# izhengfan/se2lam

Measured on AMD Instinct MI355X. Metric: BA GN-iters/s (200 KF, 20k pts), higher is better.
Workload: dtype f64; 1 GPU; globalBA-window 200 KF / 20000 landmarks / 119817 EdgeSE2XYZ + 199 PreEdgeSE2, LM optimize(10) (config 4 formulation, SURVEY D3); parallelism=single GPU

## Files before the change

experiments/chol32_emu.cpp:

```cpp
#include "waveemu.h"

#include <cmath>
#include <cstdio>
#include <cstdlib>
#include <cstring>
#include <string>
#include <vector>

using std::min;
using std::max;
#define __host__
#define WAVE_LOCKSTEP() waveemu::wave_barrier()
#define SE2_WAIT_VM6(a, b, c, d, e, f) WAIT_VM()
static inline void WAIT_VM();
struct BaCtl { int done; };
static inline double bcast_lane(double v, int lane) { return waveemu_readlane(v, lane); }
static inline d2_t load_agent(const double* p) { return d2_t{p[0], p[1]}; }
struct PendingStore { double* p; d2_t v; };
static thread_local std::vector<PendingStore> g_pending[256];
static inline void store_agent(double* p, d2_t v) { g_pending[waveemu::g()->cur].push_back(PendingStore{p, v}); }
static inline void WAIT_VM() {
    std::vector<PendingStore>& q = g_pending[waveemu::g()->cur];
    for (const PendingStore& s : q) { s.p[0] = s.v.x; s.p[1] = s.v.y; }
    q.clear();
// ... 30 lines not shown
    std::printf("n = %d%s: ld %d, %d tile rows, %d block columns (%d on the longest chain), %d tasks of 256 threads\n", S.n, nd ? " (two arcs + separator)" : "", S.ld,
                S.nt, S.nbc, S.chain, ntask);
    std::vector<double> PUB(2 * (size_t)S.nt * S.nbc * kSlabs * kSlabDoubles + S.ld, 0.0), x(S.n, 0.0);
    std::vector<unsigned> flagA((size_t)S.nt * S.nbc * kSlabs, 0u), flagR((size_t)S.nt * S.nbc * kSlabs, 0u);
    double fail = 0.0;
    int rc = 0, same = 0;
    std::vector<double> x_first;
    for (unsigned seed = seed0; seed < seed0 + nseeds; ++seed) {
        std::fill(PUB.begin(), PUB.end(), 0.0);
        std::fill(x.begin(), x.end(), 0.0);
        double* YU = PUB.data() + 2 * (size_t)S.nt * S.nbc * kSlabs * kSlabDoubles;
        unsigned epoch = seed;
        unsigned long long sw = 0;
        static unsigned long long head = 0;
        auto task = [&]() {
            d_chol_tiles<false>(blockIdx.x, S.A.data(), PUB.data(), YU, S.ld, S.n, S.nbc, S.plan.tasks.data(), S.plan.deps.data(), nullptr, flagA.data(), flagR.data(),
                                &epoch, &fail, nullptr, nullptr, x.data(), nullptr, &head, ntask);
            WAIT_VM();
        };
        if (resident > 0)
            waveemu::run_grid(256, ntask, resident, seed, task);
        else
            for (int t = 0; t < ntask; ++t) sw += waveemu::run_group(256, t, ntask, seed * 7919u + t, task);
        const double res = chol_residual(S, x);
        std::printf("interleaving %u: %llu switches, |A x - b|_inf / |b|_inf = %.3e %s, failure flag %g\n", seed, sw, res, res < 1e-11 ? "(ok)" : "(MISMATCH)", fail);
        if (indefinite) {
            std::printf("  (indefinite system: the failure flag is %s)\n", fail == 1.0 ? "raised, as it must be" : "NOT raised");
            return fail == 1.0 ? 0 : 1;
        }
        if (!(res < 1e-11) || fail != 0.0) rc = 1;
        if (x_first.empty()) x_first = x;
// ... 7 lines not shown
```

experiments/waveemu/chol_host.h:

```cpp
#pragma once
#include <algorithm>
#include <cstdio>
#include <vector>

struct Plan {
    std::vector<int4> tasks;
    std::vector<int> deps;
};

inline Plan plan_from_pattern(std::vector<std::vector<char>> P, int nt, int nbc, int* chain_len) {
    for (int m = 0; m < nbc; ++m)
        for (int j = m + 1; j < nbc; ++j)
            if (P[j][m])
                for (int i = j; i < nt; ++i)
                    if (P[i][m]) P[i][j] = 1;
    std::vector<std::vector<char>> R(nbc, std::vector<char>(nbc, 0));
    for (int r = 0; r < nbc; ++r) {
        R[r][r] = 1;
        for (int j = r + 1; j < nbc; ++j)
            for (int m = r; m < j; ++m)
                if (R[r][m] && P[j][m]) { R[r][j] = 1; break; }
    }
    Plan p;
    auto add = [&](int kind, int i, int j, const std::vector<int>& d) {
        int4 t;
        t.x = i | (kind << 16); t.y = j; t.z = (int)p.deps.size();
        p.deps.insert(p.deps.end(), d.begin(), d.end());
        t.w = (int)p.deps.size();
        p.tasks.push_back(t);
    };
    std::vector<int> depth(nbc, 1);
    for (int j = 0; j < nbc; ++j) {
        for (int m = 0; m < j; ++m)
            if (P[j][m]) depth[j] = std::max(depth[j], depth[m] + 1);
        for (int i = j; i < nt; ++i) {
            if (i > j && !P[i][j]) continue;
            std::vector<int> d;
            for (int m = 0; m < j; ++m)
                if (P[j][m]) d.push_back(m | (i != j && P[i][m] ? 1 << 15 : 0));
            add(0, i, j, d);
        }
        for (int r = 0; r < j; ++r) {
            if (!R[r][j]) continue;
            std::vector<int> d;
            for (int m = 0; m < j; ++m)
                if (P[j][m]) d.push_back(m | (m >= r && R[r][m] ? 1 << 15 : 0));
            add(1, r, j, d);
        }
    }
    for (int r = 0; r < nbc; ++r) {
        std::vector<int> d;
        for (int j = r; j < nbc; ++j)
            if (R[r][j]) d.push_back(j);
        add(2, r, 0, d);
    }
    *chain_len = *std::max_element(depth.begin(), depth.end());
    return p;
}

struct CholSystem {
    int n, ld, nt, nbc, chain;
    std::vector<double> A, b;
    Plan plan;
};
inline CholSystem chol_system(int NB, int n_dense, int arc, int sep) {
    CholSystem S;
    const bool nd = arc > 0;
    const int n = S.n = nd ? NB * (2 * arc + sep) : n_dense;
    const int ld = S.ld = ((n + 1 + NB - 1) / NB) * NB, nt = S.nt = ld / NB, nbc = S.nbc = (n + NB - 1) / NB;
    std::vector<std::vector<char>> P(nt, std::vector<char>(nbc, 1));
    if (nd)
// ... 26 lines not shown
                if (S.A[(size_t)r * ld + c] != 0.0) { std::printf("the arcs are coupled?\n"); std::abort(); }
    S.plan = plan_from_pattern(P, nt, nbc, &S.chain);
    return S;
}
inline bool chol_system_from_file(int NB, const char* path, CholSystem& S) {
    FILE* f = std::fopen(path, "rb");
    int hdr[4];
    if (!f || std::fread(hdr, 4, 4, f) != 4) return false;
    S.n = hdr[0]; S.ld = hdr[1]; S.nt = S.ld / NB; S.nbc = (S.n + NB - 1) / NB; S.chain = 0;
    S.plan.tasks.resize(hdr[2]); S.plan.deps.resize(hdr[3]); S.A.resize((size_t)S.ld * S.ld); S.b.resize(S.n);
    bool ok = std::fread(S.plan.tasks.data(), sizeof(int4), hdr[2], f) == (size_t)hdr[2];
    ok = ok && std::fread(S.plan.deps.data(), 4, hdr[3], f) == (size_t)hdr[3];
    ok = ok && std::fread(S.A.data(), 8, S.A.size(), f) == S.A.size();
    std::fclose(f);
    for (int c = 0; ok && c < S.n; ++c) S.b[c] = S.A[(size_t)S.n * S.ld + c];
    return ok;
}
inline double chol_residual(const CholSystem& S, const std::vector<double>& x) {
    double worst = 0.0, scale = 0.0;
    for (int r = 0; r < S.n; ++r) {
        double a = -S.b[r];
        for (int c = 0; c < S.n; ++c) a += S.A[(size_t)r * S.ld + c] * x[c];
        if (!(std::fabs(a) <= worst)) worst = std::fabs(a);
        scale = std::fmax(scale, std::fabs(S.b[r]));
    }
    return worst / scale;
}
```

include/se2gpu.h:

```cpp
#ifndef SE2GPU_H
#define SE2GPU_H

#include <stddef.h>
#include <stdint.h>

#ifdef __cplusplus
extern "C" {
#endif

#define SE2GPU_OK 0
#define SE2GPU_ERR_INVALID (-1)
#define SE2GPU_ERR_NO_DEVICE (-2)
#define SE2GPU_ERR_HIP (-3)
#define SE2GPU_ERR_CAPACITY (-4)
#define SE2GPU_ERR_STATE (-5)

const char* se2gpu_last_error(void);
int se2gpu_device_count(void);
const char* se2gpu_version(void);

typedef struct se2gpu_orb se2gpu_orb;

typedef struct se2gpu_orb_params {
    int32_t nfeatures;
// ... 173 lines not shown
int se2gpu_ba_get_se2(se2gpu_ba* h, int id, double xyt[3]);
int se2gpu_ba_get_xyz(se2gpu_ba* h, int id, double xyz[3]);
int se2gpu_ba_get_all(se2gpu_ba* h, double* poses , double* lms );
double se2gpu_ba_chi2(se2gpu_ba* h);

int se2gpu_ba_debug_reduced_system(se2gpu_ba* h, double lambda, double* S, double* bs);
int se2gpu_ba_debug_solve(se2gpu_ba* h, double lambda, double* x, int* factor_ok);
int se2gpu_ba_debug_solver_path(const se2gpu_ba* h);
int se2gpu_ba_debug_linearize_counts(const se2gpu_ba* h, int* runs, int* skips, long long* twin_bytes);
int se2gpu_ba_debug_pool_sizes(int out2[2]);
int se2gpu_ba_debug_chol_verify(se2gpu_ba* h, unsigned long long* counts2, unsigned long long* records, int cap);
int se2gpu_ba_debug_solve_plan(int P, int D, const uint8_t* pattern, int allow_nd, int* nsys, int* nbc, int* depth, int* ntask,
                               int* ndep, int32_t* pose_off, int32_t* tasks4, int task_cap, int32_t* deps, int dep_cap);
int se2gpu_ba_debug_solve_plan_tile(int P, int D, const uint8_t* pattern, int allow_nd, int tile, int* nsys, int* nbc, int* depth, int* ntask,
                                    int* ndep, int32_t* pose_off, int32_t* tasks4, int task_cap, int32_t* deps, int dep_cap);

int se2gpu_triangulate(int n, const se2gpu_keypoint* kps_ref, const se2gpu_keypoint* kps_cur, int n_cur,
                       int32_t* match_idx, const uint8_t* has_observation, const float* P_ref, const float* P_cur,
                       const float* Ocam, float lower_depth, float upper_depth, int min_degree, float* pos_out,
                       uint8_t* good_parallax, int* n_good, int* n_tracked_old);

typedef struct se2gpu_track se2gpu_track;
int se2gpu_track_create(se2gpu_track** out);
void se2gpu_track_destroy(se2gpu_track* h);
int se2gpu_track_fundamental_mask(se2gpu_track* h, const float* pt1, const float* pt2, int n, uint8_t* mask,
                                  int* n_inliers);
int se2gpu_track_remove_outliers(se2gpu_track* h, const se2gpu_keypoint* kps1, int n1, const se2gpu_keypoint* kps2,
                                 int n2, int32_t* matches, int* n_inliers);
int se2gpu_track_last_ransac(const se2gpu_track* h, int info[4]);
int se2gpu_track_triangulate(se2gpu_track* h, int n, const se2gpu_keypoint* kps_ref, const se2gpu_keypoint* kps_cur,
// ... 103 lines not shown
```

se2lam_amd/capi.py:

```python
from __future__ import annotations

import ctypes as C
import os

import numpy as np

HERE = os.path.dirname(os.path.abspath(__file__))
LIB_PATH = os.path.join(HERE, "lib", "libse2gpu.so")

OK = 0
ERR_INVALID, ERR_NO_DEVICE, ERR_HIP, ERR_CAPACITY, ERR_STATE = -1, -2, -3, -4, -5


class Se2GpuError(RuntimeError):
    def __init__(self, code, msg):
        super().__init__(f"se2gpu error {code}: {msg}")
        self.code = code


class Keypoint(C.Structure):
    _fields_ = [("x", C.c_float), ("y", C.c_float), ("size", C.c_float), ("angle", C.c_float),
                ("response", C.c_float), ("octave", C.c_int32), ("class_id", C.c_int32)]


# ... 125 lines not shown
    "se2gpu_ba_optimize": (_I, [_VP, _I, _I, _PU8, _I, C.POINTER(BaStats)]),
    "se2gpu_ba_optimize_batch": (_I, [C.POINTER(_VP), _I, _I, _I, _PU8, C.POINTER(BaStats)]),
    "se2gpu_ba_last_batch_path": (_I, []),
    "se2gpu_ba_get_se2": (_I, [_VP, _I, _PD]),
    "se2gpu_ba_get_xyz": (_I, [_VP, _I, _PD]),
    "se2gpu_ba_get_all": (_I, [_VP, _PD, _PD]),
    "se2gpu_ba_chi2": (_D, [_VP]),
    "se2gpu_ba_debug_reduced_system": (_I, [_VP, _D, _PD, _PD]),
    "se2gpu_ba_debug_solve": (_I, [_VP, _D, _PD, C.POINTER(C.c_int)]),
    "se2gpu_ba_debug_solver_path": (_I, [_VP]),
    "se2gpu_ba_debug_linearize_counts": (_I, [_VP, C.POINTER(C.c_int), C.POINTER(C.c_int), C.POINTER(C.c_longlong)]),
    "se2gpu_ba_debug_chol_verify": (_I, [_VP, _VP, _VP, _I]),
    "se2gpu_ba_debug_pool_sizes": (_I, [_VP]),
    "se2gpu_ba_debug_solve_plan": (_I, [_I, _I, _VP, _I, _VP, _VP, _VP, _VP, _VP, _VP, _VP, _I, _VP, _I]),
    "se2gpu_ba_debug_solve_plan_tile": (_I, [_I, _I, _VP, _I, _I, _VP, _VP, _VP, _VP, _VP, _VP, _VP, _I, _VP, _I]),
    "se2gpu_triangulate": (_I, [_I, _VP, _VP, _I, _VP, _VP, _VP, _VP, _VP, C.c_float, C.c_float, _I, _VP, _VP,
                           C.POINTER(C.c_int), C.POINTER(C.c_int)]),
    "se2gpu_track_create": (_I, [C.POINTER(_VP)]),
    "se2gpu_track_destroy": (None, [_VP]),
    "se2gpu_track_fundamental_mask": (_I, [_VP, _VP, _VP, _I, _VP, C.POINTER(C.c_int)]),
    "se2gpu_track_remove_outliers": (_I, [_VP, _VP, _I, _VP, _I, _VP, C.POINTER(C.c_int)]),
    "se2gpu_track_last_ransac": (_I, [_VP, _VP]),
    "se2gpu_plane_motion_prior": (_I, [_VP, _VP, _D, _D, _D, _VP, _VP]),
    "se2gpu_track_pose_ba": (_I, [_VP, _VP, _VP, _VP, _I, _VP, _VP, _VP, _D, _D, _D, _D, _I, _VP, C.POINTER(BaStats)]),
    "se2gpu_track_triangulate": (_I, [_VP, _I, _VP, _VP, _I, _VP, _VP, _VP, _VP, _VP, C.c_float, C.c_float, _I, _VP, _VP,
                                 C.POINTER(C.c_int), C.POINTER(C.c_int)]),
    "se2gpu_ba_reduce_buffer_doubles": (_SZ, [_VP, _I]),
    "se2gpu_ba_exchange_doubles": (_SZ, [_I]),
    "se2gpu_ba_exchange_doubles_h": (_SZ, [_VP]),
    "se2gpu_ba_exchange_row": (_I, [_I, C.POINTER(C.c_size_t), C.POINTER(C.c_int)]),
# ... 187 lines not shown
```

se2lam_amd/csrc/ba.hip:

```cpp
#include <algorithm>
#include <atomic>
#include <chrono>
#include <cmath>
#include <cstdlib>
#include <functional>
#include <limits>
#include <mutex>
#include <thread>
#include <tuple>
#include <memory>
#include <unordered_map>

#include "common.h"
#include "se3_math.h"
#include "ba_device.h"
#include "ba3_device.h"
#include "ba_window.h"

using namespace se2gpu;
using namespace se2gpu::badev;

namespace {


// ... 940 lines not shown

constexpr int kVfyRecords = 64, kVfyChk = 8 + 8 * kVfyRecords;
__device__ inline unsigned long long wave_xor64(unsigned long long v) {
#pragma unroll
    for (int m = 1; m < 64; m <<= 1) v ^= (unsigned long long)__shfl_xor((long long)v, m);
    return v;
}
__device__ inline unsigned long long bits4(d2_t a, d2_t b) {
    return (unsigned long long)__double_as_longlong(a.x) ^ (unsigned long long)__double_as_longlong(a.y) ^
           (unsigned long long)__double_as_longlong(b.x) ^ (unsigned long long)__double_as_longlong(b.y);
}
template <bool VERIFY>
__device__ __forceinline__ void d_chol_tiles(const unsigned bx_dispatch, const double* __restrict__ A, double* __restrict__ PUB,
                                                     double* __restrict__ YU, int ld, int n,
                                                     int nbc, const int4* __restrict__ tasks, const int* __restrict__ deps,
                                                     const int* __restrict__ col_src,
                                                     unsigned* __restrict__ flagA, unsigned* __restrict__ flagR,
                                                     const unsigned* __restrict__ epoch_ptr, double* __restrict__ fail,
                                                     long long* __restrict__ dbg, const BaCtl* __restrict__ ctl,
                                                     double* __restrict__ xout, unsigned long long* __restrict__ vfy,
                                                     unsigned long long* __restrict__ head, int ntask) {
    if (ctl && ctl->done) return;
    __shared__ unsigned task_s;
    if (head) {
        if (threadIdx.x == 0) {
            const unsigned c = __hip_atomic_fetch_add(reinterpret_cast<unsigned*>(head), 1u, __ATOMIC_RELAXED, __HIP_MEMORY_SCOPE_AGENT);
            if (c == (unsigned)ntask - 1u) __hip_atomic_store(reinterpret_cast<unsigned*>(head), 0u, __ATOMIC_RELAXED, __HIP_MEMORY_SCOPE_AGENT);
            task_s = c;
        }
        __syncthreads();
// ... 6 lines not shown
    double (*Tb)[kNB + 2] = reinterpret_cast<double (*)[kNB + 2]>(LD);
    double (*Tc)[kNB + 2] = reinterpret_cast<double (*)[kNB + 2]>(LD + kTile);
    double (*Ta)[kNB + 2] = reinterpret_cast<double (*)[kNB + 2]>(LD + 2 * kTile);
    double (*COLV)[kNB] = reinterpret_cast<double (*)[kNB]>(LD + 3 * kTile);
    double* const DUMMY = LD + 3 * kTile + kNB * kNB;
    double (*MRC)[64] = reinterpret_cast<double (*)[64]>(LD + kTile);
    static_assert(16 * 64 <= kTile && 32 * 64 <= 2 * kTile, "rows 0..15 of MRC lie inside Tc, all of it inside Tc | Ta");
    __shared__ int ok_s, ready_s, loaded_s, slab_s[kSlabs];
    __shared__ int deps_s[64];
    const int tid = threadIdx.x;
    if (tid == 0) { ready_s = 0; loaded_s = 0; ok_s = 1; }
    if (tid < kSlabs) slab_s[tid] = 0;
    long long* stamp = dbg ? dbg + (size_t)bx * 16 : nullptr;
    if (stamp && tid == 0) stamp[0] = wall_clock64();
    const int4 tk = tasks[bx];
    if (tid < tk.w - tk.z && tid < 64) deps_s[tid] = deps[tk.z + tid];
    __syncthreads();
    if ((tk.x >> 16) == 2) {
        const int r = tk.x & 0xffff;
        const int it = n / kNB;
        const int row = tid / 8, c4 = (tid % 8) * 4;
        double acc = 0.0;
        for (int dq = tk.z; dq < tk.w; ++dq) {
            const int j = deps_s[dq - tk.z];
            if (tid == 0) {
                const bool lazy = dq + 1 < tk.w;
                bool ok = true;
                for (int sl = 0; sl < kSlabs; ++sl) {
                    ok = ok && spin_until(flagR + ((size_t)r * nbc + j) * kSlabs + sl, epoch, lazy);
                    ok = ok && spin_until((it == j ? flagR : flagA) + ((size_t)it * nbc + j) * kSlabs + sl, epoch, lazy);
// ... 37 lines not shown
#pragma unroll
    for (int v = 0; v < 4; ++v) {
        D0[v] = A[(size_t)(kNB * j + orow + 4 * v) * ld + kNB * j + ocol];
        if (!isR && !isDiag) T0[v] = A[(size_t)(kNB * i + orow + 4 * v) * ld + kNB * j + ocol];
    }
    const int sr = ln >> 1, sc = 8 * wv + 4 * (ln & 1);
    for (int dq = tk.z; dq < tk.w; ++dq) {
        const int dep = deps_s[dq - tk.z];
        const int m = dep & 0x7fff;
        const bool hasT = (dep >> 15) != 0;
        __syncthreads();
        if (!ok_s) {
            if (tid == 0) fail[0] = 1e6;
            return;
        }
        const bool lazy = dq + 1 < tk.w;
        const unsigned* f0 = flagA + ((size_t)j * nbc + m) * kSlabs + wv;
        const unsigned* f1 = hasT ? (isR ? flagR : flagA) + ((size_t)i * nbc + m) * kSlabs + wv : f0;
        const int need = dq - tk.z + 1;
        bool staged = false;
        int mult = 0;
        long long t0 = 0;
        while (mult < kSlabs) {
            unsigned v0 = 0, v1 = 0;
            if (!staged) { v0 = poll_agent(f0); v1 = poll_agent(f1); }
            bool progress = false;
            if (__hip_atomic_load(&slab_s[mult], __ATOMIC_ACQUIRE, __HIP_MEMORY_SCOPE_WORKGROUP) >= need) {
                const int k0 = 8 * mult + acol;
                const double b0 = Tb[qj + arow][k0], b1 = Tb[qj + arow][k0 + 4];
                const double c0 = Tc[qi + arow][k0], c1 = Tc[qi + arow][k0 + 4];
                const double a0 = Ta[qi + arow][k0], a1 = Ta[qi + arow][k0 + 4];
// ... 184 lines not shown
    if (!isR && i == n / kNB && lane == (isDiag ? 0 : kNB) + n % kNB) {
#pragma unroll
        for (int q = 0; q < 8; q += 2) store_agent(YU + c0 + cb + q, d2_t{m[q], m[q + 1]});
    }
    if (bad && isDiag && lane == 0) fail[0] = 1.0;
    asm volatile("s_waitcnt vmcnt(0)" ::: "memory");
    if (lane == 0)
        __hip_atomic_store((isR || isDiag ? flagR : flagA) + ((size_t)i * nbc + j) * kSlabs + w, epoch, __ATOMIC_RELAXED, __HIP_MEMORY_SCOPE_AGENT);
    if (stamp && lane == 0) stamp[12 + w] = wall_clock64();
    if (stamp && tid == 192) stamp[5] = wall_clock64();
}
template <bool VERIFY>
__global__ __launch_bounds__(256) void k_chol_tiles(const double* __restrict__ A, double* __restrict__ PUB,
                                                     double* __restrict__ YU, int ld, int n,
                                                     int nbc, const int4* __restrict__ tasks, const int* __restrict__ deps,
                                                     const int* __restrict__ col_src,
                                                     unsigned* __restrict__ flagA, unsigned* __restrict__ flagR,
                                                     const unsigned* __restrict__ epoch_ptr, double* __restrict__ fail,
                                                     long long* __restrict__ dbg, const BaCtl* __restrict__ ctl,
                                                     double* __restrict__ xout, unsigned long long* __restrict__ vfy,
                                                     unsigned long long* __restrict__ head, int ntask) {
    d_chol_tiles<VERIFY>(blockIdx.x, A, PUB, YU, ld, n, nbc, tasks, deps, col_src, flagA, flagR, epoch_ptr, fail, dbg, ctl, xout, vfy, head, ntask);
}

__global__ __launch_bounds__(256) void k_chol_apply(const double* __restrict__ A, const double* __restrict__ R, int ld,
                                                     int n, double* __restrict__ x, const BaCtl* __restrict__ ctl,
                                                     const int* __restrict__ col_src) {
    if (ctl && ctl->done) return;
    const int r = blockIdx.x * 4 + threadIdx.x / 64;
    const int lane = threadIdx.x & 63;
    if (r >= n) return;
    const double* y = A + (size_t)n * ld;
    double acc = 0.0;
    for (int c = r + lane; c < n; c += 64) acc += R[(size_t)r * ld + c] * y[c];
    acc = wave_sum(acc);
    const int dst = col_src ? col_src[r] : r;
    if (lane == 0 && dst >= 0) x[dst] = acc;
// ... 1359 lines not shown
    DevBuf<int4> grp;
    int nwg_off = 0, grp_cap_wg = 0;
    DevBuf<uint8_t> garena;
    DevBuf<int> plan_np, plan_base, plan_key0, plan_key1, plan_idx, plan_hist, plan_offs, plan_out, plan_tsum, plan_toff;
    DevBuf<int2> plan_st0, plan_st1;
    bool odo_fallback = false;
    bool odo_self_loop = false;
    DevBuf<double> e_uv, e_info, o_meas, o_info;
    DevBuf<double> Hpl, Hpp_e, bp_e, Hll, bl, Dinv, z, Y, Dg, Hpp, bp, Oii, Ojj, Oij, obi, obj;
    DevBuf<double> red_own, xp, part, scal, diag3, Rinv;
    DevBuf<double> rec_twin;
    bool run_spec = false;
    DevBuf<double> red_packed;
    DevBuf<int4> chol_tasks;
    DevBuf<int> chol_deps;
    DevBuf<int> pose_off;
    DevBuf<int> col_src;
    std::vector<int> h_pose_off;
    DevBuf<uint8_t> plan_nz;
    DevBuf<double> plan_nzd;
    PinBuf<uint8_t> h_plan_nz;
    DevBuf<uint8_t> solver_arena;
    int nsys = 0;
    int solve_depth = 0;
    DevBuf<unsigned> chol_flags;
    DevBuf<unsigned long long> chol_head;
    DevBuf<unsigned long long> chol_vfy;
    DevBuf<int> plan_place;
    DevBuf<unsigned> fin_counter;
    DevBuf<unsigned long long> l0_acc;
// ... 542 lines not shown
            ++used;
        }
        if (used == gpw) used = 0;
    }
    flush();
    if (grp.empty()) grp.assign(gpw, make_int4(-1, 0, 0, 0));
    pl.nwg_off = (int)(grp.size() / gpw);
}

struct SolvePlan {
    int nsys = 0, nbc = 0, nt = 0, depth = 0, ntile = 0;
    bool permuted = false;
    std::vector<int> pose_off, col_src;
    std::vector<int4> tasks;
    std::vector<int> deps;
};

void solve_plan_build(int P, int D, const uint8_t* pat, const std::vector<std::vector<int>>& parts, bool pad, SolvePlan& sp, int nb = kNB) {
    sp.pose_off.assign(P, 0);
    int c = 0;
    for (const auto& part : parts) {
        for (int p : part) { sp.pose_off[p] = c; c += D; }
        if (pad) c = (c + nb - 1) / nb * nb;
    }
    sp.nsys = c;
    sp.permuted = pad;
    sp.col_src.assign(sp.nsys, -1);
    for (int p = 0; p < P; ++p)
        for (int k = 0; k < D; ++k) sp.col_src[sp.pose_off[p] + k] = D * p + k;
    const int nbc = (sp.nsys + nb - 1) / nb;
// ... 37 lines not shown
        for (int i = j + 1; i < nt; ++i) {
            if (!L(i, j)) continue;
            for (int k = i; k < nt; ++k)
                if (L(k, j) && k < nt && i < nbc) L(k, i) = 1;
        }
    std::vector<uint8_t> Rt((size_t)nbc * nbc, 0);
    auto R = [&](int r, int j) -> uint8_t& { return Rt[(size_t)r * nbc + j]; };
    for (int r = 0; r < nbc; ++r) {
        R(r, r) = 1;
        for (int j = r + 1; j < nbc; ++j)
            for (int m = r; m < j; ++m)
                if (R(r, m) && L(j, m)) { R(r, j) = 1; break; }
    }
    sp.tasks.clear();
    sp.deps.clear();
    sp.ntile = 0;
    std::vector<int> depth(nbc, 0);
    sp.depth = 0;
    for (int j = 0; j < nbc; ++j) {
        int dj = 0;
        for (int m = 0; m < j; ++m)
            if (L(j, m)) dj = std::max(dj, depth[m]);
        depth[j] = dj + 1;
        sp.depth = std::max(sp.depth, depth[j]);
        for (int i = j; i < nt; ++i) {
            if (!L(i, j)) continue;
            const int first = (int)sp.deps.size();
            for (int m = 0; m < j; ++m)
                if (L(j, m)) sp.deps.push_back(m | ((i != j && L(i, m)) ? 0x8000 : 0));
            sp.tasks.push_back(make_int4(i, j, first, (int)sp.deps.size()));
            ++sp.ntile;
        }
        for (int r = 0; r < j; ++r) {
            if (!R(r, j)) continue;
            const int first = (int)sp.deps.size();
            for (int m = 0; m < j; ++m)
                if (L(j, m)) sp.deps.push_back(m | ((m >= r && R(r, m)) ? 0x8000 : 0));
            sp.tasks.push_back(make_int4(r | (1 << 16), j, first, (int)sp.deps.size()));
            ++sp.ntile;
        }
    }
    for (int r = 0; r < nbc; ++r) {
        const int first = (int)sp.deps.size();
        for (int j = r; j < nbc; ++j)
            if (R(r, j)) sp.deps.push_back(j);
        sp.tasks.push_back(make_int4(r | (2 << 16), 0, first, (int)sp.deps.size()));
    }
}

void solve_plan_choose(int P, int D, const uint8_t* pat_in, bool allow_nd, SolvePlan& best, bool symmetric = false, int nb = kNB) {
    std::vector<int> all(P);
    for (int p = 0; p < P; ++p) all[p] = p;
    std::vector<uint8_t> sym;
    const uint8_t* pat = pat_in;
    if (pat_in && !symmetric) {
        sym.assign((size_t)P * P, 0);
        for (int a = 0; a < P; ++a)
            for (int b = 0; b < P; ++b) sym[(size_t)a * P + b] = (uint8_t)((pat_in[(size_t)a * P + b] | pat_in[(size_t)b * P + a]) != 0);
        pat = sym.data();
    }
    solve_plan_build(P, D, pat, {all}, false, best, nb);
// ... 524 lines not shown
            pat.assign((size_t)P * P, 0);
            for (int a = 0; a < P; ++a) {
                pat[(size_t)a * P + a] = 1;
                for (int b = a + 1; b < P; ++b)
                    if (nz[blk_index_of(P, a, b)]) pat[(size_t)a * P + b] = pat[(size_t)b * P + a] = 1;
            }
        }
        SolvePlan sp;
        solve_plan_choose(P, D, pat.empty() ? nullptr : pat.data(), !pat.empty(), sp, true);
        h->nsys = sp.nsys;
        h->solve_depth = sp.depth;
        h->chol_ntask = (int)sp.tasks.size();
        {
            auto up = [](size_t b) { return (b + 255) & ~(size_t)255; };
            const size_t b0 = up(sp.tasks.size() * sizeof(int4)), b1 = up(std::max<size_t>(sp.deps.size(), 1) * 4);
            const size_t b2 = sp.permuted ? up(sp.pose_off.size() * 4) : 0, b3 = sp.permuted ? up(sp.col_src.size() * 4) : 0;
            SE2_CHECK(h->h_stage_solver.reserve(std::max<size_t>(b0 + b1 + b2 + b3, (size_t)1 << 20)));
            SE2_CHECK(h->solver_arena.reserve(std::max<size_t>(b0 + b1 + b2 + b3, (size_t)1 << 20)));
            uint8_t* hp = h->h_stage_solver.p;
            std::memcpy(hp, sp.tasks.data(), sp.tasks.size() * sizeof(int4));
            std::memcpy(hp + b0, sp.deps.data(), sp.deps.size() * 4);
            if (sp.permuted) {
                std::memcpy(hp + b0 + b1, sp.pose_off.data(), sp.pose_off.size() * 4);
                std::memcpy(hp + b0 + b1 + b2, sp.col_src.data(), sp.col_src.size() * 4);
            }
            SE2_HIP(hipMemcpyAsync(h->solver_arena.p, hp, b0 + b1 + b2 + b3, hipMemcpyHostToDevice, st));
            h->chol_tasks.alias(reinterpret_cast<int4*>(h->solver_arena.p));
            h->chol_deps.alias(reinterpret_cast<int*>(h->solver_arena.p + b0));
            if (sp.permuted) {
                h->pose_off.alias(reinterpret_cast<int*>(h->solver_arena.p + b0 + b1));
                h->col_src.alias(reinterpret_cast<int*>(h->solver_arena.p + b0 + b1 + b2));
            }
        }
        if (sp.permuted) {
            h->h_pose_off = sp.pose_off;
            h->ld = ((sp.nsys + 1 + kNB - 1) / kNB) * kNB;
            const size_t nred2 = (size_t)h->ld * h->ld + 4;
            SE2_CHECK(h->red_own.reserve(nred2));
            h->red = h->red_own.p;
            SE2_CHECK(h->Rinv.reserve(chol_work_doubles(h->ld)));
            SE2_CHECK(h->xp.reserve((size_t)std::max(n, sp.nsys)));
            SE2_HIP(hipMemsetAsync(h->red, 0, nred2 * sizeof(double), st));
            hipLaunchKernelGGL(k_solver_pads, grid1((size_t)sp.nsys, 256), dim3(256), 0, st, h->red, h->ld, sp.nsys, h->col_src.p);
            SE2_HIP(hipGetLastError());
        } else {
            h->h_pose_off.clear();
// ... 345 lines not shown
    unsigned long long* const head = (2 * h->chol_ntask <= capacity) ? nullptr : h->chol_head.p;
    if (h->chol_steps) {
        for (int k = 0; k < nbc; ++k)
            SE2_LAUNCH(h->prof, st, "k_chol_step", k_chol_step, dim3(nbc - k, nt), dim3(256), 0, A, Rm, ld, n, nt, k, fail, c);
        SE2_LAUNCH(h->prof, st, "k_chol_apply", k_chol_apply, dim3((n + 3) / 4), dim3(256), 0, A, Rm, ld, n, h->xp.p, c,
                   (const int*)h->col_src.p);
    } else {
        double* YU = Rm + 2 * (size_t)nt * nbc * kSlabs * kSlabDoubles;
        unsigned* flagA = h->chol_flags.p;
        unsigned* flagR = flagA + kSlabs * (size_t)nt * nbc;
        static const bool fault = env_flag("SE2GPU_BA_CHOL_FAULT", false);
        const int skip = (fault && !h->chol_faulted && h->chol_ntask > 1) ? 1 : 0;
        h->chol_faulted = true;
        if (h->chol_vfy.p)
            SE2_LAUNCH(h->prof, st, "k_chol_tiles", k_chol_tiles<true>, dim3(h->chol_ntask - skip), dim3(256), 0, A, Rm, YU, ld, n, nbc,
                       h->chol_tasks.p + skip, (const int*)h->chol_deps.p, (const int*)h->col_src.p, flagA, flagR, &h->ctl.p->epoch,
                       fail, h->chol_trace.p, c, h->xp.p, h->chol_vfy.p, head, h->chol_ntask - skip);
        else
            SE2_LAUNCH(h->prof, st, "k_chol_tiles", k_chol_tiles<false>, dim3(h->chol_ntask - skip), dim3(256), 0, A, Rm, YU, ld, n, nbc,
                       h->chol_tasks.p + skip, (const int*)h->chol_deps.p, (const int*)h->col_src.p, flagA, flagR, &h->ctl.p->epoch,
                       fail, h->chol_trace.p, c, h->xp.p, (unsigned long long*)nullptr, head, h->chol_ntask - skip);
    }
    SE2_HIP(hipGetLastError());
    return SE2GPU_OK;
}

int ba_lambda_init(se2gpu_ba* h) {
    hipStream_t st = h->stream;
    if (h->model) {
        SE2_LAUNCH(h->prof, st, "k3_pose_diag", k3_pose_diag, grid1((size_t)h->P * 64, kBlock), dim3(kBlock), 0, h->P,
                   h->pose_ptr.p, h->pose_edges.p, h->Hpp_e.p, h->fixed.p, h->prior_has.p,
                   h->model == 2 ? h->ph.p : h->prior_info.p, h->podo_ptr.p, h->podo_item.p, h->Oii.p, h->Ojj.p, h->diag3.p);
        SE2_LAUNCH(h->prof, st, "k_maxdiag", k_maxdiag, dim3(1), dim3(1024), 0, h->L, h->Hll.p, h->P, h->diag3.p,
                   h->fixed.p, h->scal.p, 6, 0, h->ctl.p);
        SE2_HIP(hipGetLastError());
// ... 295 lines not shown
        bp.reduce2.add(((h->P + 1 + 7) & ~7) + ((h->nwg_off + 7) & ~7), h->P, h->ld, h->nwg_off, 0.0, h->root, h->grp.p, h->blk_a.p,
                       h->blk_b.p, h->pair_i.p, h->pair_j.p, h->blk_odo.p, h->Hpl.p, h->Dg.p, h->fixed.p, h->pose_ptr.p,
                       h->pose_edges.p, h->podo_ptr.p, h->podo_item.p, h->o_i.p, h->o_j.p, h->o_meas.p, h->o_info.p, B.pa, h->red,
                       h->bp.p, B.c, B.pb, &h->ctl.p->epoch, (const int*)h->pose_off.p, h->nsys, (const double*)nullptr,
                       (const double*)nullptr);
        {
            const int n = h->nsys, ld = h->ld;
            const int nt = ld / kNB, nbc = (n + kNB - 1) / kNB;
            double* Rm = h->Rinv.p;
            double* YU = Rm + 2 * (size_t)nt * nbc * kSlabs * kSlabDoubles;
            unsigned* flagA = h->chol_flags.p;
            unsigned* flagR = flagA + kSlabs * (size_t)nt * nbc;
            double* fail = h->red + (size_t)ld * ld + 2;
            bp.verify = hs[0]->chol_vfy.p != nullptr;
            if (bp.verify)
                bp.chol_v.add(h->chol_ntask, (const double*)h->red, Rm, YU, ld, n, nbc, h->chol_tasks.p, (const int*)h->chol_deps.p,
                              (const int*)h->col_src.p, flagA, flagR, &h->ctl.p->epoch,
                              fail, h->chol_trace.p, (const BaCtl*)h->ctl.p, h->xp.p, h->chol_vfy.p, h->chol_head.p, h->chol_ntask);
            else
                bp.chol.add(h->chol_ntask, (const double*)h->red, Rm, YU, ld, n, nbc, h->chol_tasks.p, (const int*)h->chol_deps.p,
                            (const int*)h->col_src.p, flagA, flagR, &h->ctl.p->epoch,
                            fail, h->chol_trace.p, (const BaCtl*)h->ctl.p, h->xp.p, (unsigned long long*)nullptr, h->chol_head.p, h->chol_ntask);
        }
    }
    bp.ctl_init.commit(bp.arena); bp.eval0.commit(bp.arena); bp.step.commit(bp.arena); bp.step_notify.commit(bp.arena);
    bp.lin0.commit(bp.arena); bp.lin.commit(bp.arena); bp.odo.commit(bp.arena); bp.pose_reduce.commit(bp.arena);
    bp.maxdiag.commit(bp.arena); bp.reduce2.commit(bp.arena);
    bp.chol.commit(bp.arena); bp.chol_v.commit(bp.arena);
    SE2_CHECK(bp.arena.dev.reserve(bp.arena.host.size()));
    SE2_HIP(hipMemcpyAsync(bp.arena.dev.p, bp.arena.host.data(), bp.arena.host.size(), hipMemcpyHostToDevice, bp.stream));
    bp.events.resize(count);
    return SE2GPU_OK;
}

int ba_batch_slot(const BatchPlan& bp, bool first, bool notify) {
// ... 685 lines not shown

int se2gpu_ba_debug_solve_plan(int P, int D, const uint8_t* pattern, int allow_nd, int* nsys, int* nbc, int* depth, int* ntask,
                               int* ndep, int32_t* pose_off, int32_t* tasks4, int task_cap, int32_t* deps, int dep_cap) {
    SE2_REQUIRE(P > 0 && (D == 3 || D == 6) && nsys && nbc && depth && ntask && ndep, SE2GPU_ERR_INVALID, "debug_solve_plan: bad argument");
    SolvePlan sp;
    solve_plan_choose(P, D, pattern, allow_nd != 0, sp);
    *nsys = sp.nsys; *nbc = sp.nbc; *depth = sp.depth; *ntask = (int)sp.tasks.size(); *ndep = (int)sp.deps.size();
    if (pose_off) std::memcpy(pose_off, sp.pose_off.data(), (size_t)P * 4);
    if (tasks4) {
        SE2_REQUIRE(task_cap >= (int)sp.tasks.size(), SE2GPU_ERR_CAPACITY, "debug_solve_plan: %zu tasks", sp.tasks.size());
        std::memcpy(tasks4, sp.tasks.data(), sp.tasks.size() * sizeof(int4));
    }
    if (deps) {
        SE2_REQUIRE(dep_cap >= (int)sp.deps.size(), SE2GPU_ERR_CAPACITY, "debug_solve_plan: %zu dependency entries", sp.deps.size());
        std::memcpy(deps, sp.deps.data(), sp.deps.size() * 4);
    }
    return SE2GPU_OK;
}

int se2gpu_ba_debug_chol_verify(se2gpu_ba* h, unsigned long long* counts2, unsigned long long* records, int cap) {
    SE2_REQUIRE(h && h->initialized && h->chol_vfy.p, SE2GPU_ERR_STATE, "the handle does not verify its hand-offs (SE2GPU_BA_CHOL_VERIFY=1)");
    SE2_CHECK(ba_join(h));
    SE2_HIP(hipStreamSynchronize(h->stream));
    unsigned long long head[8];
    SE2_HIP(hipMemcpy(head, h->chol_vfy.p, sizeof(head), hipMemcpyDeviceToHost));
    counts2[0] = head[0]; counts2[1] = head[1];
    const int nrec = (int)std::min<unsigned long long>(std::min<unsigned long long>(head[0], kVfyRecords), (unsigned long long)std::max(cap, 0));
    if (nrec && records) SE2_HIP(hipMemcpy(records, h->chol_vfy.p + 8, (size_t)nrec * 8 * sizeof(unsigned long long), hipMemcpyDeviceToHost));
    return SE2GPU_OK;
}
// ... 40 lines not shown
        std::vector<int4> tk(h->chol_ntask);
        SE2_HIP(hipMemcpy(tr.data(), h->chol_trace.p, tr.size() * sizeof(long long), hipMemcpyDeviceToHost));
        SE2_HIP(hipMemcpy(tk.data(), h->chol_tasks.p, tk.size() * sizeof(int4), hipMemcpyDeviceToHost));
        int ndep = 0;
        for (const int4& t : tk) ndep = std::max(ndep, t.w);
        std::vector<int> dp((size_t)std::max(ndep, 1));
        if (ndep) SE2_HIP(hipMemcpy(dp.data(), h->chol_deps.p, (size_t)ndep * sizeof(int), hipMemcpyDeviceToHost));
        long long t0 = tr[0];
        for (int t = 0; t < h->chol_ntask; ++t) t0 = std::min(t0, tr[16 * (size_t)t]);
        for (int t = 0; t < h->chol_ntask; ++t) {
            std::fprintf(stderr, "choltrace %d %d %d %d %d", t, tk[t].x & 0xffff, tk[t].x >> 16, tk[t].y,
                         tk[t].w > tk[t].z ? dp[tk[t].w - 1] : -1);
            for (int q = 0; q < 6; ++q) std::fprintf(stderr, " %lld", tr[16 * (size_t)t + q] ? tr[16 * (size_t)t + q] - t0 : -1);
            std::fprintf(stderr, " %lld %lld", tr[16 * (size_t)t + 6], tr[16 * (size_t)t + 7] ? tr[16 * (size_t)t + 7] - t0 : -1);
            for (int q = 8; q < 16; ++q) std::fprintf(stderr, " %lld", tr[16 * (size_t)t + q] ? tr[16 * (size_t)t + q] - t0 : -1);
            std::fprintf(stderr, "\n");
        }
    }
    return SE2GPU_OK;
}

namespace {

bool ba_env_sync() {
    static const bool on = env_flag("SE2GPU_BA_SYNC", false);
    return on;
}

int ba_run_prologue(se2gpu_ba* h, hipStream_t st, hipEvent_t* ev, int iters, int mode, bool sync, const volatile uint8_t* stop_flag) {
    SE2_CHECK(ba_join(h, st, ev));
// ... 592 lines not shown
```

se2lam_amd/optimizer.py:

```python
from __future__ import annotations

import ctypes as C
import os

import numpy as np

from . import capi

LM, GN = 0, 1


def _stats_dict(st):
    n = min(st.iterations, 64)
    return dict(iterations=st.iterations, trials=st.trials, terminated=bool(st.terminated),
                stopped=bool(st.stopped), chi2_init=st.chi2_init, chi2_final=st.chi2_final,
                lambda_final=st.lambda_final, chi2_hist=list(st.chi2_hist[:n]),
                lambda_hist=list(st.lambda_hist[:n]), trials_hist=list(st.trials_hist[:n]))


def _no_fallback(h):
    if capi.lib().se2gpu_ba_debug_solver_path(h) == 2 and os.environ.get("SE2GPU_BA_CHOL_FAULT") != "1":
        raise RuntimeError("se2gpu_ba: k_chol_tiles timed out and the handle fell back to k_chol_step")


# ... 63 lines not shown
        stop = self._stop.ctypes.data_as(C.POINTER(C.c_uint8)) if self._stop is not None else None
        capi.check(capi.lib().se2gpu_ba_optimize(self._h, int(iterations), int(mode), stop, int(self._verbose),
                                                 C.byref(st)))
        self.stats = _stats_dict(st)
        _no_fallback(self._h)
        return st.iterations

    def exchange_doubles(self) -> int:
        return int(capi.lib().se2gpu_ba_exchange_doubles_h(self._h))

    def chol_verify(self):
        counts = np.zeros(2, np.uint64)
        rec = np.zeros((64, 8), np.uint64)
        capi.check(capi.lib().se2gpu_ba_debug_chol_verify(self._h, counts.ctypes.data, rec.ctypes.data, 64))
        return int(counts[0]), int(counts[1]), rec[:min(int(counts[0]), 64)]

    def solver_path(self) -> int:
        return int(capi.lib().se2gpu_ba_debug_solver_path(self._h))

    def linearize_counts(self):
        runs, skips, twin = C.c_int(0), C.c_int(0), C.c_longlong(0)
        capi.check(capi.lib().se2gpu_ba_debug_linearize_counts(self._h, C.byref(runs), C.byref(skips), C.byref(twin)))
        return int(runs.value), int(skips.value), int(twin.value)

    def activeRobustChi2(self) -> float:
        v = capi.lib().se2gpu_ba_chi2(self._h)
        if v < 0:
            capi.check(capi.ERR_STATE)
        return float(v)

# ... 305 lines not shown
```

Baseline: 6928 iters/s.

## Order Cholesky tile dependencies by depth and apply last-level updates eagerly

The tile-Cholesky plan now sorts each column's dependency list by elimination depth and records, per task, how many trailing dependencies sit at the deepest level (neager). In the kernel the lazy/eager split uses this count, so every update from the critical-path level is applied eagerly, not only the last one. The aim is to shorten waiting on the critical chain by letting shallow dependencies be consumed first and the deepest ones as soon as they arrive. It adds a per-task int array to the solver arena and changes update order, which can change floating-point summation order.

```diff
diff --git a/experiments/chol32_emu.cpp b/experiments/chol32_emu.cpp
--- a/experiments/chol32_emu.cpp
+++ b/experiments/chol32_emu.cpp
@@ -68,7 +68,7 @@
         unsigned long long sw = 0;
         static unsigned long long head = 0;
         auto task = [&]() {
-            d_chol_tiles<false>(blockIdx.x, S.A.data(), PUB.data(), YU, S.ld, S.n, S.nbc, S.plan.tasks.data(), S.plan.deps.data(), nullptr, flagA.data(), flagR.data(),
+            d_chol_tiles<false>(blockIdx.x, S.A.data(), PUB.data(), YU, S.ld, S.n, S.nbc, S.plan.tasks.data(), S.plan.deps.data(), S.plan.neager.data(), nullptr, flagA.data(), flagR.data(),
                                 &epoch, &fail, nullptr, nullptr, x.data(), nullptr, &head, ntask);
             WAIT_VM();
         };
diff --git a/experiments/waveemu/chol_host.h b/experiments/waveemu/chol_host.h
--- a/experiments/waveemu/chol_host.h
+++ b/experiments/waveemu/chol_host.h
@@ -6,7 +6,23 @@
 struct Plan {
     std::vector<int4> tasks;
     std::vector<int> deps;
+    std::vector<int> neager;
 };
+
+inline void plan_neager(Plan& p, int nbc) {
+    std::vector<int> depth(nbc, 1);
+    for (const int4& t : p.tasks)
+        if ((t.x >> 16) == 0 && (t.x & 0xffff) == t.y)
+            for (int q = t.z; q < t.w; ++q) depth[t.y] = std::max(depth[t.y], depth[p.deps[q] & 0x7fff] + 1);
+    p.neager.clear();
+    for (const int4& t : p.tasks) {
+        int ne = 0;
+        if ((t.x >> 16) == 2) ne = 1;
+        else
+            for (int q = t.w - 1; q >= t.z && depth[p.deps[q] & 0x7fff] == depth[t.y] - 1; --q) ++ne;
+        p.neager.push_back(ne);
+    }
+}
 
 inline Plan plan_from_pattern(std::vector<std::vector<char>> P, int nt, int nbc, int* chain_len) {
     for (int m = 0; m < nbc; ++m)
@@ -33,18 +49,20 @@
     for (int j = 0; j < nbc; ++j) {
         for (int m = 0; m < j; ++m)
             if (P[j][m]) depth[j] = std::max(depth[j], depth[m] + 1);
+        std::vector<int> cols;
+        for (int m = 0; m < j; ++m)
+            if (P[j][m]) cols.push_back(m);
+        std::stable_sort(cols.begin(), cols.end(), [&](int a, int b) { return depth[a] < depth[b]; });
         for (int i = j; i < nt; ++i) {
             if (i > j && !P[i][j]) continue;
             std::vector<int> d;
-            for (int m = 0; m < j; ++m)
-                if (P[j][m]) d.push_back(m | (i != j && P[i][m] ? 1 << 15 : 0));
+            for (int m : cols) d.push_back(m | (i != j && P[i][m] ? 1 << 15 : 0));
             add(0, i, j, d);
         }
         for (int r = 0; r < j; ++r) {
             if (!R[r][j]) continue;
             std::vector<int> d;
-            for (int m = 0; m < j; ++m)
-                if (P[j][m]) d.push_back(m | (m >= r && R[r][m] ? 1 << 15 : 0));
+            for (int m : cols) d.push_back(m | (m >= r && R[r][m] ? 1 << 15 : 0));
             add(1, r, j, d);
         }
     }
@@ -55,6 +73,7 @@
         add(2, r, 0, d);
     }
     *chain_len = *std::max_element(depth.begin(), depth.end());
+    plan_neager(p, nbc);
     return p;
 }
 
@@ -111,6 +130,7 @@
     ok = ok && std::fread(S.A.data(), 8, S.A.size(), f) == S.A.size();
     std::fclose(f);
     for (int c = 0; ok && c < S.n; ++c) S.b[c] = S.A[(size_t)S.n * S.ld + c];
+    if (ok) plan_neager(S.plan, S.nbc);
     return ok;
 }
 inline double chol_residual(const CholSystem& S, const std::vector<double>& x) {
diff --git a/include/se2gpu.h b/include/se2gpu.h
--- a/include/se2gpu.h
+++ b/include/se2gpu.h
@@ -211,6 +211,8 @@
                                int* ndep, int32_t* pose_off, int32_t* tasks4, int task_cap, int32_t* deps, int dep_cap);
 int se2gpu_ba_debug_solve_plan_tile(int P, int D, const uint8_t* pattern, int allow_nd, int tile, int* nsys, int* nbc, int* depth, int* ntask,
                                     int* ndep, int32_t* pose_off, int32_t* tasks4, int task_cap, int32_t* deps, int dep_cap);
+int se2gpu_ba_debug_solve_plan_neager(int P, int D, const uint8_t* pattern, int allow_nd, int tile, int32_t* neager, int cap);
+int se2gpu_ba_debug_plan_neager(se2gpu_ba* h, int* nsys, int* permuted, int* ntask, int32_t* neager, int cap);
 
 int se2gpu_triangulate(int n, const se2gpu_keypoint* kps_ref, const se2gpu_keypoint* kps_cur, int n_cur,
                        int32_t* match_idx, const uint8_t* has_observation, const float* P_ref, const float* P_cur,
diff --git a/se2lam_amd/capi.py b/se2lam_amd/capi.py
--- a/se2lam_amd/capi.py
+++ b/se2lam_amd/capi.py
@@ -163,6 +163,8 @@
     "se2gpu_ba_debug_pool_sizes": (_I, [_VP]),
     "se2gpu_ba_debug_solve_plan": (_I, [_I, _I, _VP, _I, _VP, _VP, _VP, _VP, _VP, _VP, _VP, _I, _VP, _I]),
     "se2gpu_ba_debug_solve_plan_tile": (_I, [_I, _I, _VP, _I, _I, _VP, _VP, _VP, _VP, _VP, _VP, _VP, _I, _VP, _I]),
+    "se2gpu_ba_debug_solve_plan_neager": (_I, [_I, _I, _VP, _I, _I, _VP, _I]),
+    "se2gpu_ba_debug_plan_neager": (_I, [_VP, C.POINTER(C.c_int), C.POINTER(C.c_int), C.POINTER(C.c_int), _VP, _I]),
     "se2gpu_triangulate": (_I, [_I, _VP, _VP, _I, _VP, _VP, _VP, _VP, _VP, C.c_float, C.c_float, _I, _VP, _VP,
                            C.POINTER(C.c_int), C.POINTER(C.c_int)]),
     "se2gpu_track_create": (_I, [C.POINTER(_VP)]),
diff --git a/se2lam_amd/csrc/ba.hip b/se2lam_amd/csrc/ba.hip
--- a/se2lam_amd/csrc/ba.hip
+++ b/se2lam_amd/csrc/ba.hip
@@ -978,6 +978,7 @@
 __device__ __forceinline__ void d_chol_tiles(const unsigned bx_dispatch, const double* __restrict__ A, double* __restrict__ PUB,
                                                      double* __restrict__ YU, int ld, int n,
                                                      int nbc, const int4* __restrict__ tasks, const int* __restrict__ deps,
+                                                     const int* __restrict__ neager,
                                                      const int* __restrict__ col_src,
                                                      unsigned* __restrict__ flagA, unsigned* __restrict__ flagR,
                                                      const unsigned* __restrict__ epoch_ptr, double* __restrict__ fail,
@@ -1014,6 +1015,7 @@
     long long* stamp = dbg ? dbg + (size_t)bx * 16 : nullptr;
     if (stamp && tid == 0) stamp[0] = wall_clock64();
     const int4 tk = tasks[bx];
+    const int ne = neager[bx];
     if (tid < tk.w - tk.z && tid < 64) deps_s[tid] = deps[tk.z + tid];
     __syncthreads();
     if ((tk.x >> 16) == 2) {
@@ -1081,7 +1083,7 @@
             if (tid == 0) fail[0] = 1e6;
             return;
         }
-        const bool lazy = dq + 1 < tk.w;
+        const bool lazy = dq < tk.w - ne;
         const unsigned* f0 = flagA + ((size_t)j * nbc + m) * kSlabs + wv;
         const unsigned* f1 = hasT ? (isR ? flagR : flagA) + ((size_t)i * nbc + m) * kSlabs + wv : f0;
         const int need = dq - tk.z + 1;
@@ -1296,13 +1298,14 @@
 __global__ __launch_bounds__(256) void k_chol_tiles(const double* __restrict__ A, double* __restrict__ PUB,
                                                      double* __restrict__ YU, int ld, int n,
                                                      int nbc, const int4* __restrict__ tasks, const int* __restrict__ deps,
+                                                     const int* __restrict__ neager,
                                                      const int* __restrict__ col_src,
                                                      unsigned* __restrict__ flagA, unsigned* __restrict__ flagR,
                                                      const unsigned* __restrict__ epoch_ptr, double* __restrict__ fail,
                                                      long long* __restrict__ dbg, const BaCtl* __restrict__ ctl,
                                                      double* __restrict__ xout, unsigned long long* __restrict__ vfy,
                                                      unsigned long long* __restrict__ head, int ntask) {
-    d_chol_tiles<VERIFY>(blockIdx.x, A, PUB, YU, ld, n, nbc, tasks, deps, col_src, flagA, flagR, epoch_ptr, fail, dbg, ctl, xout, vfy, head, ntask);
+    d_chol_tiles<VERIFY>(blockIdx.x, A, PUB, YU, ld, n, nbc, tasks, deps, neager, col_src, flagA, flagR, epoch_ptr, fail, dbg, ctl, xout, vfy, head, ntask);
 }
 
 __global__ __launch_bounds__(256) void k_chol_apply(const double* __restrict__ A, const double* __restrict__ R, int ld,
@@ -2692,6 +2695,7 @@
     DevBuf<double> red_packed;
     DevBuf<int4> chol_tasks;
     DevBuf<int> chol_deps;
+    DevBuf<int> chol_neager;
     DevBuf<int> pose_off;
     DevBuf<int> col_src;
     std::vector<int> h_pose_off;
@@ -3264,6 +3268,7 @@
     std::vector<int> pose_off, col_src;
     std::vector<int4> tasks;
     std::vector<int> deps;
+    std::vector<int> neager;
 };
 
 void solve_plan_build(int P, int D, const uint8_t* pat, const std::vector<std::vector<int>>& parts, bool pad, SolvePlan& sp, int nb = kNB) {
@@ -3331,29 +3336,34 @@
     }
     sp.tasks.clear();
     sp.deps.clear();
+    sp.neager.clear();
     sp.ntile = 0;
-    std::vector<int> depth(nbc, 0);
+    std::vector<int> depth(nbc, 0), cols;
     sp.depth = 0;
     for (int j = 0; j < nbc; ++j) {
-        int dj = 0;
+        cols.clear();
         for (int m = 0; m < j; ++m)
-            if (L(j, m)) dj = std::max(dj, depth[m]);
+            if (L(j, m)) cols.push_back(m);
+        std::stable_sort(cols.begin(), cols.end(), [&](int a, int b) { return depth[a] < depth[b]; });
+        const int dj = cols.empty() ? 0 : depth[cols.back()];
+        int ne = 0;
+        for (int m : cols) ne += depth[m] == dj ? 1 : 0;
         depth[j] = dj + 1;
         sp.depth = std::max(sp.depth, depth[j]);
         for (int i = j; i < nt; ++i) {
             if (!L(i, j)) continue;
             const int first = (int)sp.deps.size();
-            for (int m = 0; m < j; ++m)
-                if (L(j, m)) sp.deps.push_back(m | ((i != j && L(i, m)) ? 0x8000 : 0));
+            for (int m : cols) sp.deps.push_back(m | ((i != j && L(i, m)) ? 0x8000 : 0));
             sp.tasks.push_back(make_int4(i, j, first, (int)sp.deps.size()));
+            sp.neager.push_back(ne);
             ++sp.ntile;
         }
         for (int r = 0; r < j; ++r) {
             if (!R(r, j)) continue;
             const int first = (int)sp.deps.size();
-            for (int m = 0; m < j; ++m)
-                if (L(j, m)) sp.deps.push_back(m | ((m >= r && R(r, m)) ? 0x8000 : 0));
+            for (int m : cols) sp.deps.push_back(m | ((m >= r && R(r, m)) ? 0x8000 : 0));
             sp.tasks.push_back(make_int4(r | (1 << 16), j, first, (int)sp.deps.size()));
+            sp.neager.push_back(ne);
             ++sp.ntile;
         }
     }
@@ -3362,6 +3372,7 @@
         for (int j = r; j < nbc; ++j)
             if (R(r, j)) sp.deps.push_back(j);
         sp.tasks.push_back(make_int4(r | (2 << 16), 0, first, (int)sp.deps.size()));
+        sp.neager.push_back(1);
     }
 }
 
@@ -3916,22 +3927,25 @@
         {
             auto up = [](size_t b) { return (b + 255) & ~(size_t)255; };
             const size_t b0 = up(sp.tasks.size() * sizeof(int4)), b1 = up(std::max<size_t>(sp.deps.size(), 1) * 4);
+            const size_t bn = up(sp.neager.size() * 4);
             const size_t b2 = sp.permuted ? up(sp.pose_off.size() * 4) : 0, b3 = sp.permuted ? up(sp.col_src.size() * 4) : 0;
-            SE2_CHECK(h->h_stage_solver.reserve(std::max<size_t>(b0 + b1 + b2 + b3, (size_t)1 << 20)));
-            SE2_CHECK(h->solver_arena.reserve(std::max<size_t>(b0 + b1 + b2 + b3, (size_t)1 << 20)));
+            SE2_CHECK(h->h_stage_solver.reserve(std::max<size_t>(b0 + b1 + bn + b2 + b3, (size_t)1 << 20)));
+            SE2_CHECK(h->solver_arena.reserve(std::max<size_t>(b0 + b1 + bn + b2 + b3, (size_t)1 << 20)));
             uint8_t* hp = h->h_stage_solver.p;
             std::memcpy(hp, sp.tasks.data(), sp.tasks.size() * sizeof(int4));
             std::memcpy(hp + b0, sp.deps.data(), sp.deps.size() * 4);
+            std::memcpy(hp + b0 + b1, sp.neager.data(), sp.neager.size() * 4);
             if (sp.permuted) {
-                std::memcpy(hp + b0 + b1, sp.pose_off.data(), sp.pose_off.size() * 4);
-                std::memcpy(hp + b0 + b1 + b2, sp.col_src.data(), sp.col_src.size() * 4);
+                std::memcpy(hp + b0 + b1 + bn, sp.pose_off.data(), sp.pose_off.size() * 4);
+                std::memcpy(hp + b0 + b1 + bn + b2, sp.col_src.data(), sp.col_src.size() * 4);
             }
-            SE2_HIP(hipMemcpyAsync(h->solver_arena.p, hp, b0 + b1 + b2 + b3, hipMemcpyHostToDevice, st));
+            SE2_HIP(hipMemcpyAsync(h->solver_arena.p, hp, b0 + b1 + bn + b2 + b3, hipMemcpyHostToDevice, st));
             h->chol_tasks.alias(reinterpret_cast<int4*>(h->solver_arena.p));
             h->chol_deps.alias(reinterpret_cast<int*>(h->solver_arena.p + b0));
+            h->chol_neager.alias(reinterpret_cast<int*>(h->solver_arena.p + b0 + b1));
             if (sp.permuted) {
-                h->pose_off.alias(reinterpret_cast<int*>(h->solver_arena.p + b0 + b1));
-                h->col_src.alias(reinterpret_cast<int*>(h->solver_arena.p + b0 + b1 + b2));
+                h->pose_off.alias(reinterpret_cast<int*>(h->solver_arena.p + b0 + b1 + bn));
+                h->col_src.alias(reinterpret_cast<int*>(h->solver_arena.p + b0 + b1 + bn + b2));
             }
         }
         if (sp.permuted) {
@@ -4307,11 +4321,11 @@
         h->chol_faulted = true;
         if (h->chol_vfy.p)
             SE2_LAUNCH(h->prof, st, "k_chol_tiles", k_chol_tiles<true>, dim3(h->chol_ntask - skip), dim3(256), 0, A, Rm, YU, ld, n, nbc,
-                       h->chol_tasks.p + skip, (const int*)h->chol_deps.p, (const int*)h->col_src.p, flagA, flagR, &h->ctl.p->epoch,
+                       h->chol_tasks.p + skip, (const int*)h->chol_deps.p, (const int*)h->chol_neager.p + skip, (const int*)h->col_src.p, flagA, flagR, &h->ctl.p->epoch,
                        fail, h->chol_trace.p, c, h->xp.p, h->chol_vfy.p, head, h->chol_ntask - skip);
         else
             SE2_LAUNCH(h->prof, st, "k_chol_tiles", k_chol_tiles<false>, dim3(h->chol_ntask - skip), dim3(256), 0, A, Rm, YU, ld, n, nbc,
-                       h->chol_tasks.p + skip, (const int*)h->chol_deps.p, (const int*)h->col_src.p, flagA, flagR, &h->ctl.p->epoch,
+                       h->chol_tasks.p + skip, (const int*)h->chol_deps.p, (const int*)h->chol_neager.p + skip, (const int*)h->col_src.p, flagA, flagR, &h->ctl.p->epoch,
                        fail, h->chol_trace.p, c, h->xp.p, (unsigned long long*)nullptr, head, h->chol_ntask - skip);
     }
     SE2_HIP(hipGetLastError());
@@ -4637,11 +4651,11 @@
             double* fail = h->red + (size_t)ld * ld + 2;
             bp.verify = hs[0]->chol_vfy.p != nullptr;
             if (bp.verify)
-                bp.chol_v.add(h->chol_ntask, (const double*)h->red, Rm, YU, ld, n, nbc, h->chol_tasks.p, (const int*)h->chol_deps.p,
+                bp.chol_v.add(h->chol_ntask, (const double*)h->red, Rm, YU, ld, n, nbc, h->chol_tasks.p, (const int*)h->chol_deps.p, (const int*)h->chol_neager.p,
                               (const int*)h->col_src.p, flagA, flagR, &h->ctl.p->epoch,
                               fail, h->chol_trace.p, (const BaCtl*)h->ctl.p, h->xp.p, h->chol_vfy.p, h->chol_head.p, h->chol_ntask);
             else
-                bp.chol.add(h->chol_ntask, (const double*)h->red, Rm, YU, ld, n, nbc, h->chol_tasks.p, (const int*)h->chol_deps.p,
+                bp.chol.add(h->chol_ntask, (const double*)h->red, Rm, YU, ld, n, nbc, h->chol_tasks.p, (const int*)h->chol_deps.p, (const int*)h->chol_neager.p,
                             (const int*)h->col_src.p, flagA, flagR, &h->ctl.p->epoch,
                             fail, h->chol_trace.p, (const BaCtl*)h->ctl.p, h->xp.p, (unsigned long long*)nullptr, h->chol_head.p, h->chol_ntask);
         }
@@ -5357,6 +5371,27 @@
     if (deps) {
         SE2_REQUIRE(dep_cap >= (int)sp.deps.size(), SE2GPU_ERR_CAPACITY, "debug_solve_plan: %zu dependency entries", sp.deps.size());
         std::memcpy(deps, sp.deps.data(), sp.deps.size() * 4);
+    }
+    return SE2GPU_OK;
+}
+
+int se2gpu_ba_debug_solve_plan_neager(int P, int D, const uint8_t* pattern, int allow_nd, int tile, int32_t* neager, int cap) {
+    SE2_REQUIRE(P > 0 && (D == 3 || D == 6) && (tile == 32 || tile == 64) && neager, SE2GPU_ERR_INVALID, "debug_solve_plan_neager: bad argument");
+    SolvePlan sp;
+    solve_plan_choose(P, D, pattern, allow_nd != 0, sp, false, tile);
+    SE2_REQUIRE(cap >= (int)sp.neager.size(), SE2GPU_ERR_CAPACITY, "debug_solve_plan_neager: %zu tasks", sp.neager.size());
+    std::memcpy(neager, sp.neager.data(), sp.neager.size() * 4);
+    return SE2GPU_OK;
+}
+
+int se2gpu_ba_debug_plan_neager(se2gpu_ba* h, int* nsys, int* permuted, int* ntask, int32_t* neager, int cap) {
+    SE2_REQUIRE(h && h->initialized && nsys && permuted && ntask, SE2GPU_ERR_STATE, "debug_plan_neager before initialize");
+    SE2_CHECK(ba_join(h));
+    SE2_HIP(hipStreamSynchronize(h->stream));
+    *nsys = h->nsys; *permuted = h->col_src.p ? 1 : 0; *ntask = h->chol_ntask;
+    if (neager) {
+        SE2_REQUIRE(cap >= h->chol_ntask && h->chol_neager.p, SE2GPU_ERR_CAPACITY, "debug_plan_neager: %d tasks", h->chol_ntask);
+        SE2_HIP(hipMemcpy(neager, h->chol_neager.p, (size_t)h->chol_ntask * 4, hipMemcpyDeviceToHost));
     }
     return SE2GPU_OK;
 }
@@ -5427,6 +5462,14 @@
             for (int q = 0; q < 6; ++q) std::fprintf(stderr, " %lld", tr[16 * (size_t)t + q] ? tr[16 * (size_t)t + q] - t0 : -1);
             std::fprintf(stderr, " %lld %lld", tr[16 * (size_t)t + 6], tr[16 * (size_t)t + 7] ? tr[16 * (size_t)t + 7] - t0 : -1);
             for (int q = 8; q < 16; ++q) std::fprintf(stderr, " %lld", tr[16 * (size_t)t + q] ? tr[16 * (size_t)t + q] - t0 : -1);
+            std::fprintf(stderr, "\n");
+        }
+        std::vector<int> ne(h->chol_ntask);
+        SE2_HIP(hipMemcpy(ne.data(), h->chol_neager.p, ne.size() * sizeof(int), hipMemcpyDeviceToHost));
+        for (int t = 0; t < h->chol_ntask; ++t) {
+            if ((tk[t].x >> 16) == 2 || ne[t] < 2) continue;
+            std::fprintf(stderr, "choleager %d", t);
+            for (int q = tk[t].w - ne[t]; q < tk[t].w; ++q) std::fprintf(stderr, " %d", dp[q]);
             std::fprintf(stderr, "\n");
         }
     }
diff --git a/se2lam_amd/optimizer.py b/se2lam_amd/optimizer.py
--- a/se2lam_amd/optimizer.py
+++ b/se2lam_amd/optimizer.py
@@ -101,6 +101,13 @@
         rec = np.zeros((64, 8), np.uint64)
         capi.check(capi.lib().se2gpu_ba_debug_chol_verify(self._h, counts.ctypes.data, rec.ctypes.data, 64))
         return int(counts[0]), int(counts[1]), rec[:min(int(counts[0]), 64)]
+
+    def plan_neager(self):
+        nsys, perm, ntask = C.c_int(0), C.c_int(0), C.c_int(0)
+        capi.check(capi.lib().se2gpu_ba_debug_plan_neager(self._h, C.byref(nsys), C.byref(perm), C.byref(ntask), None, 0))
+        ne = np.zeros(max(ntask.value, 1), np.int32)
+        capi.check(capi.lib().se2gpu_ba_debug_plan_neager(self._h, C.byref(nsys), C.byref(perm), C.byref(ntask), ne.ctypes.data, len(ne)))
+        return int(nsys.value), bool(perm.value), ne[:ntask.value]
 
     def solver_path(self) -> int:
         return int(capi.lib().se2gpu_ba_debug_solver_path(self._h))
```

New measurement: 7233 iters/s (median of 6 runs). 4.4% higher.
